# MatejBevec/gcn-song-embeddings

Hardware: AMD Instinct MI355X
Metric: PinSAGE train-step nodes/sec (2-hop, batch 512) at 1/2/4/8 MI355X (higher is better)
Workload: dtype f32

## Files before the change

### gcn-song-embeddings_amd/csrc/conv.hip

```cpp
#include "common.h"
#include "conv.h"
#include "bf16split.h"

#include <algorithm>
#include <climits>

namespace ps {

__device__ __forceinline__ int32_t rank_in(const unsigned long long* bits, const uint32_t* prefix,
                                           int64_t v) {
  const unsigned long long w = bits[v >> 6];
  return (int32_t)(prefix[v >> 6] + __popcll(w & ((1ull << (v & 63)) - 1ull)));
}

__global__ void layer_prep_kernel(LayerPreps a) {
  const int T = a.T;
  const int64_t g0 = (int64_t)blockIdx.x * blockDim.x + threadIdx.x, gs = (int64_t)gridDim.x * blockDim.x;
  for (int l = 0; l < a.n; ++l) {
    const LayerPrep& p = a.L[l];
    if (p.z) {
      const int64_t zn4 = (int64_t)(*p.z_rows) * p.z_n / 4;
      float4* z4 = reinterpret_cast<float4*>(p.z);
      for (int64_t i = g0; i < zn4; i += gs) z4[i] = make_float4(0.f, 0.f, 0.f, 0.f);
    }
// ... 383 lines not shown
  extern __shared__ int hist[];
  const int64_t n = (int64_t)(*nS) * T;
  const int U = *nN;
  const int ns = *nsplit;
  for (int si = blockIdx.x; si < ns; si += gridDim.x) {
    const int2 sp = split[si];
    const int v = off[sp.x + 1] - off[sp.x], nc = n_chunks(v);
    for (int j = threadIdx.x; j < nc; j += blockDim.x)
      chunks[sp.y + j] = make_int2(sp.x, min(kDqChunk, v - j * kDqChunk) | kDqSplit);
  }
  if (U <= kLdsRows) {
    for (int u = threadIdx.x; u < U; u += blockDim.x) hist[u] = 0;
    __syncthreads();
    const int64_t per = (n + gridDim.x - 1) / gridDim.x;
    const int64_t e0 = (int64_t)blockIdx.x * per, e1 = min(n, e0 + per);
    for (int64_t e = e0 + threadIdx.x; e < e1; e += blockDim.x) atomicAdd(hist + loc[e], 1);
    __syncthreads();
    for (int u = threadIdx.x; u < U; u += blockDim.x)
      if (hist[u]) hist[u] = atomicAdd(cursor + u, hist[u]);
    __syncthreads();
    for (int64_t e = e0 + threadIdx.x; e < e1; e += blockDim.x) {
      const int32_t u = loc[e];
      const int pos = atomicAdd(hist + u, 1);
      put_occ(occ2, off, cbase, wloc, T, u, pos, e);
    }
    return;
  }
  const int R = (U + kLdsRows - 1) / kLdsRows;
  if (R <= max_ranges) {
    const int64_t S = max((int64_t)1, (int64_t)(2 * gridDim.x + R - 1) / R);
    const int64_t slice = (n + S - 1) / S;
    const int64_t items = (int64_t)R * S;
    for (int64_t it = blockIdx.x; it < items; it += gridDim.x) {
      const int r = (int)(it % R);
      const int u0 = r * kLdsRows, nu = min(kLdsRows, U - u0);
      const int64_t e0 = (it / R) * slice, e1 = min(n, e0 + slice);
      for (int u = threadIdx.x; u < nu; u += blockDim.x) hist[u] = 0;
      __syncthreads();
      for (int64_t e = e0 + threadIdx.x; e < e1; e += blockDim.x) {
        const int u = loc[e] - u0;
        if ((unsigned)u < (unsigned)nu) atomicAdd(hist + u, 1);
      }
      __syncthreads();
      for (int u = threadIdx.x; u < nu; u += blockDim.x)
        if (hist[u]) hist[u] = atomicAdd(cursor + u0 + u, hist[u]);
      __syncthreads();
      for (int64_t e = e0 + threadIdx.x; e < e1; e += blockDim.x) {
        const int u = loc[e] - u0;
        if ((unsigned)u < (unsigned)nu) {
          const int pos = atomicAdd(hist + u, 1);
          put_occ(occ2, off, cbase, wloc, T, u0 + u, pos, e);
        }
      }
      __syncthreads();
    }
    return;
  }
  const int lane = threadIdx.x & 63;
  for (int64_t base = ((int64_t)blockIdx.x * blockDim.x + threadIdx.x) & ~63LL; base < n;
       base += (int64_t)gridDim.x * blockDim.x) {
    const int64_t e = base + lane;
    const int32_t u = e < n ? loc[e] : -1;
    unsigned long long rem = __ballot(e < n);
    int pos = 0;
    while (rem) {
      const int leader = __ffsll((long long)rem) - 1;
      const int32_t v = __shfl(u, leader, 64);
      const unsigned long long m = __ballot(u == v);
      int b = 0;
      if (lane == leader) b = atomicAdd(cursor + v, __popcll(m));
      b = __shfl(b, leader, 64);
      if (u == v) pos = b + __popcll(m & ((1ull << lane) - 1));
      rem &= ~m;
    }
    if (e < n) put_occ(occ2, off, cbase, wloc, T, u, pos, e);
  }
}

constexpr int kSortWaveRow = 64;
__global__ __launch_bounds__(256) void csr_sort_chunks_kernel(const int2* __restrict__ chunks,
                                                              const int* __restrict__ nchunks,
                                                              const int* __restrict__ off,
                                                              int2* __restrict__ occ2) {
  const int lane = threadIdx.x & 63;
  const int64_t nw = ((int64_t)gridDim.x * blockDim.x) >> 6;
  const int nch = *nchunks;
  for (int64_t ci = ((int64_t)blockIdx.x * blockDim.x + threadIdx.x) >> 6; ci < nch; ci += nw) {
    const int2 dsc = chunks[ci];
    const int n = dsc.y & 0xff;
    if (dsc.y & kDqSplit) {
      if (ci > 0 && chunks[ci - 1].x == dsc.x) continue;
      const int nr = off[dsc.x + 1] - off[dsc.x];
      if (nr > kSortWaveRow) continue;
      const int2 v = lane < nr ? occ2[ci * kDqChunk + lane] : make_int2(INT_MAX, 0);
      int r = 0;
      for (int j = 0; j < nr; ++j) r += __shfl(v.x, j, 64) < v.x;
      __builtin_amdgcn_wave_barrier();
      if (lane < nr) occ2[ci * kDqChunk + r] = v;
      continue;
    }
    if (n < 2) continue;
    int2 v = make_int2(INT_MAX, 0);
    if (lane < n) v = occ2[ci * kDqChunk + lane];
#pragma unroll
    for (int k = 2; k <= kDqChunk; k <<= 1)
#pragma unroll
      for (int j = k >> 1; j > 0; j >>= 1) {
        const int ox = __shfl_xor(v.x, j, 64), oy = __shfl_xor(v.y, j, 64);
        const bool lower = (lane & j) == 0, up = (lane & k) == 0;
        const bool take = (lower == up) ? (ox < v.x) : (ox > v.x);
        if (take) v = make_int2(ox, oy);
      }
    if (lane < n) occ2[ci * kDqChunk + lane] = v;
  }
}

constexpr int kRankWords = 16384;
constexpr int64_t kRankBits = (int64_t)kRankWords * 32;
constexpr int kRankLds = kRankWords * 4 * 2 + 64;
__global__ __launch_bounds__(1024) void csr_sort_rows_kernel(const int2* __restrict__ split,
                                                             const int* __restrict__ nsplit,
                                                             const int* __restrict__ off, int2* __restrict__ occ2,
                                                             int2* __restrict__ tmp) {
  extern __shared__ unsigned rk[];
  unsigned* bits = rk;
  unsigned* pref = rk + kRankWords;
  int* red = reinterpret_cast<int*>(pref + kRankWords);
  const int tid = threadIdx.x, lane = tid & 63, wv = tid >> 6;
  const int ns = *nsplit;
  for (int si = blockIdx.x; si < ns; si += gridDim.x) {
    const int2 sp = split[si];
    const int n = off[sp.x + 1] - off[sp.x];
    if (n <= kSortWaveRow) continue;
    int2* row = occ2 + (int64_t)sp.y * kDqChunk;
    int2* out = tmp + (int64_t)sp.y * kDqChunk;
    int lo = INT_MAX, hi = -1;
    for (int i = tid; i < n; i += blockDim.x) {
      const int f = row[i].x;
      lo = min(lo, f);
      hi = max(hi, f);
    }
    for (int o = 32; o > 0; o >>= 1) {
      lo = min(lo, __shfl_xor(lo, o, 64));
      hi = max(hi, __shfl_xor(hi, o, 64));
    }
    if (lane == 0) red[wv] = lo;
    __syncthreads();
    if (tid == 0) {
      int a = red[0];
      for (int w = 1; w < 16; ++w) a = min(a, red[w]);
      red[0] = a;
    }
    __syncthreads();
    lo = red[0];
    __syncthreads();
    if (lane == 0) red[wv] = hi;
    __syncthreads();
    if (tid == 0) {
      int a = red[0];
      for (int w = 1; w < 16; ++w) a = max(a, red[w]);
      red[0] = a;
    }
    __syncthreads();
    hi = red[0];
    __syncthreads();
    int base = 0;
    for (int64_t w0 = lo; w0 <= hi; w0 += kRankBits) {
      const int nwords = (int)min((int64_t)kRankWords, (hi - w0) / 32 + 1);
      for (int i = tid; i < nwords; i += blockDim.x) bits[i] = 0u;
      __syncthreads();
      for (int i = tid; i < n; i += blockDim.x) {
        const int64_t b = (int64_t)row[i].x - w0;
        if (b >= 0 && b < (int64_t)nwords * 32) atomicOr(bits + (b >> 5), 1u << (b & 31));
      }
      __syncthreads();
      const int per = (nwords + (int)blockDim.x - 1) / (int)blockDim.x;
      const int i0 = tid * per;
      int s = 0;
      for (int i = i0; i < min(nwords, i0 + per); ++i) s += __popc(bits[i]);
      int inc = s;
      for (int o = 1; o < 64; o <<= 1) {
        const int y = __shfl_up(inc, o, 64);
        if (lane >= o) inc += y;
      }
      if (lane == 63) red[wv] = inc;
      __syncthreads();
      int pre = inc - s;
      for (int w = 0; w < wv; ++w) pre += red[w];
      int total = 0;
      for (int w = 0; w < 16; ++w) total += red[w];
      for (int i = i0; i < min(nwords, i0 + per); ++i) {
        pref[i] = (unsigned)pre;
        pre += __popc(bits[i]);
      }
      __syncthreads();
      for (int i = tid; i < n; i += blockDim.x) {
        const int2 v = row[i];
        const int64_t b = (int64_t)v.x - w0;
        if (b >= 0 && b < (int64_t)nwords * 32) {
          const int wd = (int)(b >> 5);
          const int r = base + (int)pref[wd] + __popc(bits[wd] & ((1u << (b & 31)) - 1u));
          out[r] = v;
        }
      }
      base += total;
      __syncthreads();
    }
    __threadfence_block();
    __syncthreads();
    for (int i = tid; i < n; i += blockDim.x) row[i] = out[i];
    __syncthreads();
  }
}

typedef int dq_v4i __attribute__((ext_vector_type(4)));
__device__ __forceinline__ void dq_store_planes(uint16_t* __restrict__ base, int64_t ps, int64_t e, float4 v) {
  float a = v.x, b = v.y, c = v.z, d = v.w;
  asm("" : "+v"(a), "+v"(b), "+v"(c), "+v"(d));
  unsigned h0, m0, l0, h1, m1, l1;
  split_pair(f32x2{a, b}, h0, m0, l0);
  split_pair(f32x2{c, d}, h1, m1, l1);
  *reinterpret_cast<uint2*>(base + e) = make_uint2(h0, h1);
  *reinterpret_cast<uint2*>(base + ps + e) = make_uint2(m0, m1);
  *reinterpret_cast<uint2*>(base + 2 * ps + e) = make_uint2(l0, l1);
}
__device__ __forceinline__ void dq_st_wt(float* row, int i, float4 v) {
  const __amdgpu_buffer_rsrc_t rs = __builtin_amdgcn_make_buffer_rsrc(row, 0, 0x7fffffff, 0x00020000);
  const dq_v4i w{__float_as_int(v.x), __float_as_int(v.y), __float_as_int(v.z), __float_as_int(v.w)};
  __builtin_amdgcn_raw_buffer_store_b128(w, rs, (unsigned)i * 16u, 0, 16);
}
__device__ __forceinline__ float4 dq_ld_wt(const float* row, int i) {
  const __amdgpu_buffer_rsrc_t rs =
      __builtin_amdgcn_make_buffer_rsrc(const_cast<float*>(row), 0, 0x7fffffff, 0x00020000);
  const dq_v4i y = __builtin_amdgcn_raw_buffer_load_b128(rs, (unsigned)i * 16u, 0, 16);
  return make_float4(__int_as_float(y.x), __int_as_float(y.y), __int_as_float(y.z), __int_as_float(y.w));
}
template <int VEC, bool PL3>
__device__ __forceinline__ void dq_tree_leaf(float4 (&acc)[VEC], const float4 (&qv)[VEC], int u, int64_t ci,
                                             int lane, int h4, int hid, const int* __restrict__ off,
                                             const int* __restrict__ cbase, int* __restrict__ tk,
                                             int64_t tk_stride, float* __restrict__ part,
                                             float* __restrict__ dpq, uint16_t* __restrict__ dpq3,
                                             int64_t ps3) {
  const int k = n_chunks(off[u + 1] - off[u]);
  const int64_t cb = cbase[u];
  int64_t g = ci - cb, span = 1, nodes = k;
  float* leaf = part + (int64_t)__builtin_amdgcn_readfirstlane((int)ci) * hid;
#pragma unroll
  for (int v = 0; v < VEC; ++v)
    if (v * 64 + lane < h4) dq_st_wt(leaf, v * 64 + lane, acc[v]);
  for (int L = 0;; ++L) {
    asm volatile("s_waitcnt vmcnt(0)" ::: "memory");
    const int64_t gp = g >> 3;
    const int nch = (int)min<int64_t>(8, nodes - 8 * gp);
    int t = 0;
    if (lane == 0) t = __hip_atomic_fetch_add(tk + L * tk_stride + cb + gp, 1, __ATOMIC_RELAXED,
                                              __HIP_MEMORY_SCOPE_AGENT);
    t = __shfl(t, 0, 64);
    if (t != nch - 1) return;
    if (lane == 0) __hip_atomic_store(tk + L * tk_stride + cb + gp, 0, __ATOMIC_RELAXED, __HIP_MEMORY_SCOPE_AGENT);
    __builtin_amdgcn_fence(__ATOMIC_ACQUIRE, "wavefront");
    float4 x[8][VEC];
#pragma unroll
    for (int c = 0; c < 8; ++c) {
      const int cc = c < nch ? c : nch - 1;
      const float* row = part + (cb + span * (8 * gp + cc)) * hid;
#pragma unroll
      for (int v = 0; v < VEC; ++v) x[c][v] = dq_ld_wt(row, min(v * 64 + lane, h4 - 1));
    }
#pragma unroll
    for (int v = 0; v < VEC; ++v) acc[v] = x[0][v];
#pragma unroll
    for (int c = 1; c < 8; ++c)
      if (c < nch)
#pragma unroll
        for (int v = 0; v < VEC; ++v) {
          acc[v].x += x[c][v].x;
          acc[v].y += x[c][v].y;
          acc[v].z += x[c][v].z;
          acc[v].w += x[c][v].w;
        }
    span *= 8;
    nodes = (nodes + 7) >> 3;
    g = gp;
    if (nodes == 1) {
      float4* o = reinterpret_cast<float4*>(dpq + (int64_t)u * hid);
#pragma unroll
      for (int v = 0; v < VEC; ++v)
        if (v * 64 + lane < h4) {
          const float4 r = make_float4(acc[v].x * lrelu_grad(qv[v].x), acc[v].y * lrelu_grad(qv[v].y),
                                       acc[v].z * lrelu_grad(qv[v].z), acc[v].w * lrelu_grad(qv[v].w));
          if (PL3) dq_store_planes(dpq3, ps3, (int64_t)u * hid + 4 * (v * 64 + lane), r);
          else o[v * 64 + lane] = r;
        }
      return;
    }
    float* node = part + (int64_t)__builtin_amdgcn_readfirstlane((int)(cb + span * g)) * hid;
#pragma unroll
    for (int v = 0; v < VEC; ++v)
      if (v * 64 + lane < h4) dq_st_wt(node, v * 64 + lane, acc[v]);
  }
}

template <int VEC, bool CM = false, bool TREE = false, bool PL3 = false>
__global__ __launch_bounds__(256) void dq_chunk_kernel(
    const int2* __restrict__ chunks, const int* __restrict__ nchunks, const int2* __restrict__ occ2,
    const float* __restrict__ dagg, int64_t ld_dagg, const float* __restrict__ q, int hid,
    float* __restrict__ dpq, float* __restrict__ part, const int32_t* __restrict__ q_src = nullptr,
    int32_t* __restrict__ csrc = nullptr, const int* __restrict__ off = nullptr,
    const int* __restrict__ cbase = nullptr, int* __restrict__ tk = nullptr, int64_t tk_stride = 0,
    uint16_t* __restrict__ dpq3 = nullptr, int64_t ps3 = 0) {
  const int lane = threadIdx.x & 63;
  const int64_t wid = ((int64_t)blockIdx.x * blockDim.x + threadIdx.x) >> 6;
  const int64_t nw = ((int64_t)gridDim.x * blockDim.x) >> 6;
  const int h4 = hid >> 2;
  const int nch = *nchunks;
  int2 dsc = make_int2(0, 0), oc = make_int2(0, 0);
  if (wid < nch) {
    dsc = chunks[wid];
    if (lane < kDqChunk) oc = occ2[wid * kDqChunk + lane];
  }
  if (!CM && h4 <= 64 * VEC) {
    float4 pend[VEC];
    float4* pend_o = nullptr;
    int64_t pend_e = -1;
    auto store_pend = [&]() __attribute__((always_inline)) {
      if (PL3 && pend_e >= 0) {
#pragma unroll
        for (int v = 0; v < VEC; ++v)
          if (v * 64 + lane < h4) dq_store_planes(dpq3, ps3, pend_e + 4 * (v * 64 + lane), pend[v]);
        pend_e = -1;
      } else if (pend_o) {
#pragma unroll
        for (int v = 0; v < VEC; ++v)
          if (v * 64 + lane < h4) pend_o[v * 64 + lane] = pend[v];
        pend_o = nullptr;
      }
    };
    for (int64_t ci = wid; ci < nch; ci += nw) {
      int2 dsc_n = make_int2(0, 0), oc_n = make_int2(0, 0);
      if (ci + nw < nch) {
        dsc_n = chunks[ci + nw];
        if (lane < kDqChunk) oc_n = occ2[(ci + nw) * kDqChunk + lane];
      }
      const int u = dsc.x, n = dsc.y & 0xff;
      const bool split = (dsc.y & kDqSplit) != 0;
      const int32_t my_row = oc.x;
      const float my_w = __int_as_float(oc.y);
      float4 qv[VEC], x[kDqChunk][VEC];
#pragma unroll
      for (int v = 0; v < VEC; ++v) qv[v] = reinterpret_cast<const float4*>(q + (int64_t)u * hid)[min(v * 64 + lane, h4 - 1)];
      const int ng = (n + 3) >> 2;
#pragma unroll
      for (int g = 0; g < kDqChunk / 4; ++g) {
        if (g < ng) {
#pragma unroll
          for (int jj = 0; jj < 4; ++jj) {
            const int j = 4 * g + jj;
            const int32_t row = __shfl(my_row, min(j, n - 1), 64);
            const float4* dr = reinterpret_cast<const float4*>(dagg + (int64_t)row * ld_dagg);
#pragma unroll
            for (int v = 0; v < VEC; ++v) x[j][v] = dr[min(v * 64 + lane, h4 - 1)];
          }
        }
      }
      store_pend();
      float4 acc[VEC];
#pragma unroll
      for (int v = 0; v < VEC; ++v) acc[v] = make_float4(0.f, 0.f, 0.f, 0.f);
#pragma unroll
      for (int g = 0; g < kDqChunk / 4; ++g) {
        if (g < ng) {
#pragma unroll
          for (int jj = 0; jj < 4; ++jj) {
            const int j = 4 * g + jj;
            const float w = j < n ? __shfl(my_w, j, 64) : 0.f;
#pragma unroll
            for (int v = 0; v < VEC; ++v) {
              acc[v].x = fmaf(w, x[j][v].x, acc[v].x);
              acc[v].y = fmaf(w, x[j][v].y, acc[v].y);
              acc[v].z = fmaf(w, x[j][v].z, acc[v].z);
              acc[v].w = fmaf(w, x[j][v].w, acc[v].w);
            }
          }
        }
      }
      if (TREE && split) {
        dq_tree_leaf<VEC, PL3>(acc, qv, u, ci, lane, h4, hid, off, cbase, tk, tk_stride, part, dpq, dpq3, ps3);
        dsc = dsc_n;
        oc = oc_n;
        continue;
      }
#pragma unroll
      for (int v = 0; v < VEC; ++v)
        pend[v] = split ? acc[v]
                        : make_float4(acc[v].x * lrelu_grad(qv[v].x), acc[v].y * lrelu_grad(qv[v].y),
                                      acc[v].z * lrelu_grad(qv[v].z), acc[v].w * lrelu_grad(qv[v].w));
      if (PL3 && !split) pend_e = (int64_t)u * hid;
      else pend_o = reinterpret_cast<float4*>(split ? part + ci * hid : dpq + (int64_t)u * hid);
      dsc = dsc_n;
      oc = oc_n;
    }
    store_pend();
    return;
  }
  for (int64_t ci = wid; ci < nch; ci += nw) {
    int2 dsc_n = make_int2(0, 0), oc_n = make_int2(0, 0);
    if (ci + nw < nch) {
      dsc_n = chunks[ci + nw];
      if (lane < kDqChunk) oc_n = occ2[(ci + nw) * kDqChunk + lane];
    }
    const int u = dsc.x, n = dsc.y & 0xff;
    const bool split = !CM && (dsc.y & kDqSplit) != 0;
    if (CM && lane == 0) csrc[ci] = q_src[u];
    const int32_t my_row = oc.x;
    const float my_w = __int_as_float(oc.y);
    for (int c0 = 0; c0 < h4; c0 += 64 * VEC) {
      float4 qv[VEC], x[kDqChunk][VEC];
#pragma unroll
      for (int v = 0; v < VEC; ++v) {
        const int c = min(c0 + v * 64 + lane, h4 - 1);
        qv[v] = reinterpret_cast<const float4*>(q + (int64_t)u * hid)[c];
      }
      const int ng = (n + 3) >> 2;
#pragma unroll
      for (int g = 0; g < kDqChunk / 4; ++g) {
        if (g < ng) {
#pragma unroll
          for (int jj = 0; jj < 4; ++jj) {
            const int j = 4 * g + jj;
            const int32_t row = __shfl(my_row, min(j, n - 1), 64);
            const float4* dr = reinterpret_cast<const float4*>(dagg + (int64_t)row * ld_dagg);
#pragma unroll
            for (int v = 0; v < VEC; ++v) x[j][v] = dr[min(c0 + v * 64 + lane, h4 - 1)];
          }
        }
      }
      float4 acc[VEC];
#pragma unroll
      for (int v = 0; v < VEC; ++v) acc[v] = make_float4(0.f, 0.f, 0.f, 0.f);
#pragma unroll
      for (int g = 0; g < kDqChunk / 4; ++g) {
        if (g < ng) {
#pragma unroll
          for (int jj = 0; jj < 4; ++jj) {
            const int j = 4 * g + jj;
            const float w = j < n ? __shfl(my_w, j, 64) : 0.f;
#pragma unroll
            for (int v = 0; v < VEC; ++v) {
              acc[v].x = fmaf(w, x[j][v].x, acc[v].x);
              acc[v].y = fmaf(w, x[j][v].y, acc[v].y);
              acc[v].z = fmaf(w, x[j][v].z, acc[v].z);
              acc[v].w = fmaf(w, x[j][v].w, acc[v].w);
            }
          }
        }
      }
      float4* o = reinterpret_cast<float4*>(split || CM ? part + ci * hid : dpq + (int64_t)u * hid);
#pragma unroll
      for (int v = 0; v < VEC; ++v) {
        const int c = c0 + v * 64 + lane;
        if (c < h4)
          o[c] = split ? acc[v]
                       : make_float4(acc[v].x * lrelu_grad(qv[v].x), acc[v].y * lrelu_grad(qv[v].y),
                                     acc[v].z * lrelu_grad(qv[v].z), acc[v].w * lrelu_grad(qv[v].w));
      }
    }
    dsc = dsc_n;
    oc = oc_n;
  }
}

constexpr int kCombWaves = 16;
__global__ __launch_bounds__(1024) void dq_combine_kernel(const int2* __restrict__ split,
                                                          const int* __restrict__ nsplit,
                                                          const int* __restrict__ off,
                                                          const float* __restrict__ part,
                                                          const float* __restrict__ q, int hid,
                                                          float* __restrict__ dpq) {
  __shared__ float4 red[kCombWaves][64];
  const int lane = threadIdx.x & 63, wv = threadIdx.x >> 6;
  const int h4 = hid >> 2;
  const int ns = *nsplit;
  for (int si = blockIdx.x; si < ns; si += gridDim.x) {
    const int2 sp = split[si];
    const int u = sp.x;
    const int64_t ci = sp.y;
    const int k = (off[u + 1] - off[u] + kDqChunk - 1) / kDqChunk;
    for (int c0 = 0; c0 < h4; c0 += 64) {
      const int c = c0 + lane;
      const int cc = min(c, h4 - 1);
      float4 acc = make_float4(0.f, 0.f, 0.f, 0.f);
      int j = wv;
      for (; j + 7 * kCombWaves < k; j += 8 * kCombWaves) {
        float4 x[8];
#pragma unroll
        for (int i = 0; i < 8; ++i)
          x[i] = reinterpret_cast<const float4*>(part + (ci + j + i * kCombWaves) * hid)[cc];
#pragma unroll
        for (int i = 0; i < 8; ++i) {
          acc.x += x[i].x;
          acc.y += x[i].y;
          acc.z += x[i].z;
          acc.w += x[i].w;
        }
      }
      for (; j < k; j += kCombWaves) {
        const float4 x = reinterpret_cast<const float4*>(part + (ci + j) * hid)[cc];
        acc.x += x.x;
        acc.y += x.y;
        acc.z += x.z;
        acc.w += x.w;
      }
      red[wv][lane] = acc;
      __syncthreads();
      if (wv == 0 && c < h4) {
        float4 t = red[0][lane];
        for (int i = 1; i < kCombWaves; ++i) {
          const float4 x = red[i][lane];
          t.x += x.x;
          t.y += x.y;
          t.z += x.z;
          t.w += x.w;
        }
        const float4 qq = reinterpret_cast<const float4*>(q + (int64_t)u * hid)[c];
        reinterpret_cast<float4*>(dpq + (int64_t)u * hid)[c] =
            make_float4(t.x * lrelu_grad(qq.x), t.y * lrelu_grad(qq.y), t.z * lrelu_grad(qq.z),
                        t.w * lrelu_grad(qq.w));
      }
      __syncthreads();
    }
  }
}

__global__ __launch_bounds__(256) void norm_lrelu_bwd_kernel(const float* __restrict__ y,
                                                             const float* __restrict__ nrm,
                                                             const float* __restrict__ dy, int n,
                                                             const int* __restrict__ nrows,
                                                             int64_t n_static,
                                                             float* __restrict__ dp,
                                                             float* __restrict__ z, int z_n,
                                                             const int* __restrict__ z_rows,
                                                             int* __restrict__ zi, int64_t zi_n) {
  const int64_t gt = (int64_t)blockIdx.x * blockDim.x + threadIdx.x;
  const int64_t gs = (int64_t)gridDim.x * blockDim.x;
  const int64_t R = nrows ? (int64_t)*nrows : n_static;
  const int lane = threadIdx.x & 63;
  const int64_t wid = ((int64_t)blockIdx.x * blockDim.x + threadIdx.x) >> 6;
  const int64_t nw = ((int64_t)gridDim.x * blockDim.x) >> 6;
  for (int64_t r = wid; r < R; r += nw) {
    float dot = 0.f;
    for (int c = lane; c < n; c += 64) dot += y[r * n + c] * dy[r * n + c];
    dot = wave_sum(dot);
    const float inv = 1.f / nrm[r];
    for (int c = lane; c < n; c += 64) {
      const float yy = y[r * n + c];
      dp[r * n + c] = lrelu_grad(yy) * (dy[r * n + c] - yy * dot) * inv;
    }
  }
  if (z) {
    const int64_t zn = (int64_t)(*z_rows) * z_n;
    for (int64_t i = gt; i < zn; i += gs) z[i] = 0.f;
  }
  if (zi)
    for (int64_t i = gt; i < zi_n; i += gs) zi[i] = 0;
}

__global__ __launch_bounds__(256) void l2norm_rows_kernel(float* __restrict__ y, int64_t n, int out,
                                                          float* __restrict__ norms) {
  const int lane = threadIdx.x & 63;
  const int64_t wid = ((int64_t)blockIdx.x * blockDim.x + threadIdx.x) >> 6;
  const int64_t nw = ((int64_t)gridDim.x * blockDim.x) >> 6;
  for (int64_t r = wid; r < n; r += nw) {
    float s2 = 0.f;
    for (int c = lane; c < out; c += 64) s2 += y[r * out + c] * y[r * out + c];
    const float nrm = sqrtf(wave_sum(s2));
    for (int c = lane; c < out; c += 64) y[r * out + c] = y[r * out + c] / nrm;
    if (lane == 0 && norms) norms[r] = nrm;
  }
}

int launch_l2norm_rows(float* y, int64_t n, int out, float* norms, hipStream_t st) {
  if (n <= 0) return kOk;
  hipLaunchKernelGGL(l2norm_rows_kernel, dim3(grid_for(n * 64, 256, 4096)), dim3(256), 0, st, y, n, out, norms);
  PS_CHECK_LAUNCH();
  return kOk;
}

constexpr int kPosCsrMax = 16384;
constexpr int kPosDig = 7, kPosBuckets = 1 << kPosDig, kPosWaves = 16;
constexpr int kPosCsrLds = 2 * kPosCsrMax * 4 + kPosBuckets * kPosWaves * 4 + 64;
__device__ __forceinline__ unsigned long long match_digit(int dig, bool valid) {
  unsigned long long m = __ballot(valid);
#pragma unroll
  for (int bit = 0; bit < kPosDig; ++bit) {
    const unsigned long long bb = __ballot((dig >> bit) & 1);
    m &= ((dig >> bit) & 1) ? bb : ~bb;
  }
  return m;
}
__global__ __launch_bounds__(1024) void pos_csr_kernel(const int32_t* __restrict__ pos_rank, int n,
                                                       const int* __restrict__ nS, int* __restrict__ rank_off,
                                                       int32_t* __restrict__ pos_sorted) {
  extern __shared__ unsigned pk[];
  if (n > kPosCsrMax) {
    if (threadIdx.x == 0) rank_off[0] = -1;
    return;
  }
  unsigned* src = pk;
  unsigned* dst = pk + kPosCsrMax;
  int* base = reinterpret_cast<int*>(pk + 2 * kPosCsrMax);
  int* wsum = base + kPosBuckets * kPosWaves;
  const int tid = threadIdx.x, lane = tid & 63, wv = tid >> 6;
  for (int i = tid; i < n; i += blockDim.x) src[i] = ((unsigned)pos_rank[i] << 16) | (unsigned)i;
  const int seg = ((n + kPosWaves - 1) / kPosWaves + 63) & ~63;
  const int w0 = min(n, wv * seg), w1 = min(n, w0 + seg);
  const unsigned long long below = (1ull << lane) - 1ull;
  for (int pass = 0; pass < 2; ++pass) {
    const int sh = 16 + kPosDig * pass;
    for (int i = tid; i < kPosBuckets * kPosWaves; i += blockDim.x) base[i] = 0;
    __syncthreads();
    for (int i0 = w0; i0 < w1; i0 += 64) {
      const int i = i0 + lane;
      const bool valid = i < w1;
      const int dig = valid ? (int)(src[i] >> sh) & (kPosBuckets - 1) : 0;
      const unsigned long long m = match_digit(dig, valid);
      if (valid && (m & below) == 0) base[dig * kPosWaves + wv] += __popcll(m);
    }
    __syncthreads();
    const int c0 = base[2 * tid], c1 = base[2 * tid + 1];
    int inc = c0 + c1;
    for (int o = 1; o < 64; o <<= 1) {
      const int y = __shfl_up(inc, o, 64);
      if (lane >= o) inc += y;
    }
    if (lane == 63) wsum[wv] = inc;
    __syncthreads();
    int pre = inc - c0 - c1;
    for (int w = 0; w < wv; ++w) pre += wsum[w];
    base[2 * tid] = pre;
    base[2 * tid + 1] = pre + c0;
    __syncthreads();
    for (int i0 = w0; i0 < w1; i0 += 64) {
      const int i = i0 + lane;
      const bool valid = i < w1;
      const unsigned key = valid ? src[i] : 0u;
      const int dig = (int)(key >> sh) & (kPosBuckets - 1);
      const unsigned long long m = match_digit(dig, valid);
      const int b = valid ? base[dig * kPosWaves + wv] : 0;
      __builtin_amdgcn_wave_barrier();
      if (valid) {
        dst[b + __popcll(m & below)] = key;
        if ((m & below) == 0) base[dig * kPosWaves + wv] = b + __popcll(m);
      }
      __builtin_amdgcn_wave_barrier();
    }
    __syncthreads();
    unsigned* t = src;
    src = dst;
    dst = t;
  }
  for (int i = tid; i < n; i += blockDim.x) {
    const unsigned v = src[i];
    const int r = (int)(v >> 16);
    pos_sorted[i] = (int32_t)(v & 0xffffu);
    const int rp = i == 0 ? -1 : (int)(src[i - 1] >> 16);
    for (int q = rp + 1; q <= r; ++q) rank_off[q] = i;
  }
  const int qe = max(*nS, (int)(src[n - 1] >> 16) + 1);
  for (int q = (int)(src[n - 1] >> 16) + 1 + tid; q <= qe; q += blockDim.x) rank_off[q] = n;
}

int launch_pos_csr(const int32_t* pos_rank, int64_t n, const int* nS, int* rank_off, int32_t* pos_sorted,
                   hipStream_t st) {
  static bool prepared = false;
  if (!prepared) {
    PS_CHECK_HIP(hipFuncSetAttribute((const void*)pos_csr_kernel, hipFuncAttributeMaxDynamicSharedMemorySize,
                                     kPosCsrLds));
    prepared = true;
  }
  if (n <= 0) return kOk;
  hipLaunchKernelGGL(pos_csr_kernel, dim3(1), dim3(1024), n <= kPosCsrMax ? (unsigned)kPosCsrLds : 0u, st, pos_rank,
                     (int)std::min<int64_t>(n, INT32_MAX), nS, rank_off, pos_sorted);
  PS_CHECK_LAUNCH();
  return kOk;
}

__device__ __forceinline__ int det_mode(int ro0, int a0, int a1) { return ro0 < 0 ? -1 : a1 - a0 == 1 ? 0 : 1; }
template <int XPL>
__device__ __forceinline__ void det_put(const float (&x)[XPL], int d, int p, int r, int grp, int mode,
                                        float* __restrict__ G, int64_t S_max, float* __restrict__ Gp, int lane) {
  float* g = G + ((int64_t)grp * S_max + r) * d;
  if (mode < 0) {
#pragma unroll
    for (int i = 0; i < XPL; ++i)
      if (lane + 64 * i < d) atomicAdd(g + lane + 64 * i, x[i]);
    return;
  }
  float* dst = mode == 0 ? g : Gp + (int64_t)p * d;
#pragma unroll
  for (int i = 0; i < XPL; ++i)
    if (lane + 64 * i < d) dst[lane + 64 * i] = x[i];
}

constexpr int kRepBatch = 16;
template <int XPL, int NG>
__global__ __launch_bounds__(256) void rep_sum_kernel(const int* __restrict__ rank_off,
                                                      const int32_t* __restrict__ pos_sorted,
                                                      const int* __restrict__ nS, int d,
                                                      const float* __restrict__ Gp, float* __restrict__ G,
                                                      int64_t S_max) {
  if (rank_off[0] < 0) return;
  const int lane = threadIdx.x & 63;
  const int64_t nw = ((int64_t)gridDim.x * blockDim.x) >> 6;
  const int64_t R = *nS;
  for (int64_t r = ((int64_t)blockIdx.x * blockDim.x + threadIdx.x) >> 6; r < R; r += nw) {
    const int o0 = rank_off[r], o1 = rank_off[r + 1];
    if (o1 - o0 < 2) continue;
    float acc[NG][XPL];
    bool any[NG];
#pragma unroll
    for (int c = 0; c < NG; ++c) {
      any[c] = false;
#pragma unroll
      for (int i = 0; i < XPL; ++i) acc[c][i] = 0.f;
    }
    for (int o = o0; o < o1; o += kRepBatch) {
      const int my_q = lane < kRepBatch && o + lane < o1 ? pos_sorted[o + lane] : -1;
      int q[kRepBatch];
      float v[kRepBatch][XPL];
#pragma unroll
      for (int u = 0; u < kRepBatch; ++u) q[u] = __shfl(my_q, u, 64);
#pragma unroll
      for (int u = 0; u < kRepBatch; ++u)
#pragma unroll
        for (int i = 0; i < XPL; ++i)
          v[u][i] = q[u] >= 0 && lane + 64 * i < d ? Gp[(int64_t)q[u] * d + lane + 64 * i] : 0.f;
#pragma unroll
      for (int u = 0; u < kRepBatch; ++u) {
        if (q[u] < 0) continue;
        const int c = NG == 1 ? 0 : q[u] % NG;
#pragma unroll
        for (int cc = 0; cc < NG; ++cc)
          if (cc == c) {
            any[cc] = true;
#pragma unroll
            for (int i = 0; i < XPL; ++i) acc[cc][i] += v[u][i];
          }
      }
    }
#pragma unroll
    for (int c = 0; c < NG; ++c)
      if (any[c]) {
        float* g = G + ((int64_t)c * S_max + r) * d;
#pragma unroll
        for (int i = 0; i < XPL; ++i)
          if (lane + 64 * i < d) g[lane + 64 * i] = acc[c][i];
      }
  }
}
// ... 794 lines not shown
```

Measured before the change: 4.154 million.

## Double-buffer dq chunk row loads and specialize on group count

Rewrites the dq chunk accumulation as a helper that keeps only two groups of four gathered rows in registers. It issues the next group's loads while FMAs run on the current group, and dispatches on the group count so each variant is fully unrolled without runtime branches. Row indices and weights move to scalar readlane/readfirstlane instead of shfl, and launch bounds now request higher occupancy. The aim is to cut VGPR pressure and hide gather latency; the risk is register spills under the tighter bound or a worse schedule from the sched barriers.

```diff
diff --git a/gcn-song-embeddings_amd/csrc/conv.hip b/gcn-song-embeddings_amd/csrc/conv.hip
--- a/gcn-song-embeddings_amd/csrc/conv.hip
+++ b/gcn-song-embeddings_amd/csrc/conv.hip
@@ -709,8 +709,69 @@
   }
 }
 
+template <int VEC, int NG, class F>
+__device__ __forceinline__ void dq_chunk_sum(float4 (&acc)[VEC], const float* __restrict__ dagg, int64_t ld_dagg,
+                                             int2 oc, int n, int c0, int lane, int h4, F&& behind_loads) {
+  float4 x[2][4][VEC];
+  unsigned col[VEC];
+  const int wbits = lane < n ? oc.y : 0;
+#pragma unroll
+  for (int v = 0; v < VEC; ++v) col[v] = 16u * (unsigned)min(c0 + v * 64 + lane, h4 - 1);
+  auto issue = [&](int g) __attribute__((always_inline)) {
+#pragma unroll
+    for (int jj = 0; jj < 4; ++jj) {
+      const int32_t row = __builtin_amdgcn_readlane(oc.x, min(4 * g + jj, n - 1));
+      const char* dr = reinterpret_cast<const char*>(dagg + (int64_t)row * ld_dagg);
+#pragma unroll
+      for (int v = 0; v < VEC; ++v) x[g & 1][jj][v] = *reinterpret_cast<const float4*>(dr + col[v]);
+    }
+  };
+  issue(0);
+  if (NG > 1) issue(1);
+  behind_loads();
+#pragma unroll
+  for (int v = 0; v < VEC; ++v) acc[v] = make_float4(0.f, 0.f, 0.f, 0.f);
+#pragma unroll
+  for (int g = 0; g < NG; ++g) {
+#pragma unroll
+    for (int jj = 0; jj < 4; ++jj) {
+      const float w = __int_as_float(__builtin_amdgcn_readlane(wbits, 4 * g + jj));
+#pragma unroll
+      for (int v = 0; v < VEC; ++v) {
+        acc[v].x = fmaf(w, x[g & 1][jj][v].x, acc[v].x);
+        acc[v].y = fmaf(w, x[g & 1][jj][v].y, acc[v].y);
+        acc[v].z = fmaf(w, x[g & 1][jj][v].z, acc[v].z);
+        acc[v].w = fmaf(w, x[g & 1][jj][v].w, acc[v].w);
+      }
+    }
+    if (g + 2 < NG) {
+#pragma unroll
+      for (int v = 0; v < VEC; ++v)
+        asm volatile("" : "+v"(acc[v].x), "+v"(acc[v].y), "+v"(acc[v].z), "+v"(acc[v].w), "+v"(col[v]));
+      issue(g + 2);
+      __builtin_amdgcn_sched_barrier(0);
+    }
+  }
+}
+template <int VEC, class F>
+__device__ __forceinline__ void dq_chunk_sum_n(float4 (&acc)[VEC], const float* __restrict__ dagg, int64_t ld_dagg,
+                                               int2 oc, int n, int c0, int lane, int h4, F&& behind_loads) {
+  static_assert(kDqChunk <= 16 && kDqChunk % 4 == 0, "dq: chunks are 1 to 4 groups of 4 rows");
+  switch ((n + 3) >> 2) {
+    case 0:
+#pragma unroll
+      for (int v = 0; v < VEC; ++v) acc[v] = make_float4(0.f, 0.f, 0.f, 0.f);
+      behind_loads();
+      break;
+    case 1: dq_chunk_sum<VEC, 1>(acc, dagg, ld_dagg, oc, n, c0, lane, h4, behind_loads); break;
+    case 2: dq_chunk_sum<VEC, 2>(acc, dagg, ld_dagg, oc, n, c0, lane, h4, behind_loads); break;
+    case 3: dq_chunk_sum<VEC, 3>(acc, dagg, ld_dagg, oc, n, c0, lane, h4, behind_loads); break;
+    default: dq_chunk_sum<VEC, 4>(acc, dagg, ld_dagg, oc, n, c0, lane, h4, behind_loads); break;
+  }
+}
+
 template <int VEC, bool CM = false, bool TREE = false, bool PL3 = false>
-__global__ __launch_bounds__(256) void dq_chunk_kernel(
+__global__ __launch_bounds__(256, (PL3 && VEC > 1) ? 3 : 4) void dq_chunk_kernel(
     const int2* __restrict__ chunks, const int* __restrict__ nchunks, const int2* __restrict__ occ2,
     const float* __restrict__ dagg, int64_t ld_dagg, const float* __restrict__ q, int hid,
     float* __restrict__ dpq, float* __restrict__ part, const int32_t* __restrict__ q_src = nullptr,
@@ -718,7 +779,8 @@
     const int* __restrict__ cbase = nullptr, int* __restrict__ tk = nullptr, int64_t tk_stride = 0,
     uint16_t* __restrict__ dpq3 = nullptr, int64_t ps3 = 0) {
   const int lane = threadIdx.x & 63;
-  const int64_t wid = ((int64_t)blockIdx.x * blockDim.x + threadIdx.x) >> 6;
+  const int64_t wid =
+      __builtin_amdgcn_readfirstlane((int)(((int64_t)blockIdx.x * blockDim.x + threadIdx.x) >> 6));
   const int64_t nw = ((int64_t)gridDim.x * blockDim.x) >> 6;
   const int h4 = hid >> 2;
   const int nch = *nchunks;
@@ -750,48 +812,13 @@
         dsc_n = chunks[ci + nw];
         if (lane < kDqChunk) oc_n = occ2[(ci + nw) * kDqChunk + lane];
       }
-      const int u = dsc.x, n = dsc.y & 0xff;
-      const bool split = (dsc.y & kDqSplit) != 0;
-      const int32_t my_row = oc.x;
-      const float my_w = __int_as_float(oc.y);
-      float4 qv[VEC], x[kDqChunk][VEC];
+      const int u = __builtin_amdgcn_readfirstlane(dsc.x), dy = __builtin_amdgcn_readfirstlane(dsc.y);
+      const int n = dy & 0xff;
+      const bool split = (dy & kDqSplit) != 0;
+      float4 qv[VEC], acc[VEC];
 #pragma unroll
       for (int v = 0; v < VEC; ++v) qv[v] = reinterpret_cast<const float4*>(q + (int64_t)u * hid)[min(v * 64 + lane, h4 - 1)];
-      const int ng = (n + 3) >> 2;
-#pragma unroll
-      for (int g = 0; g < kDqChunk / 4; ++g) {
-        if (g < ng) {
-#pragma unroll
-          for (int jj = 0; jj < 4; ++jj) {
-            const int j = 4 * g + jj;
-            const int32_t row = __shfl(my_row, min(j, n - 1), 64);
-            const float4* dr = reinterpret_cast<const float4*>(dagg + (int64_t)row * ld_dagg);
-#pragma unroll
-            for (int v = 0; v < VEC; ++v) x[j][v] = dr[min(v * 64 + lane, h4 - 1)];
-          }
-        }
-      }
-      store_pend();
-      float4 acc[VEC];
-#pragma unroll
-      for (int v = 0; v < VEC; ++v) acc[v] = make_float4(0.f, 0.f, 0.f, 0.f);
-#pragma unroll
-      for (int g = 0; g < kDqChunk / 4; ++g) {
-        if (g < ng) {
-#pragma unroll
-          for (int jj = 0; jj < 4; ++jj) {
-            const int j = 4 * g + jj;
-            const float w = j < n ? __shfl(my_w, j, 64) : 0.f;
-#pragma unroll
-            for (int v = 0; v < VEC; ++v) {
-              acc[v].x = fmaf(w, x[j][v].x, acc[v].x);
-              acc[v].y = fmaf(w, x[j][v].y, acc[v].y);
-              acc[v].z = fmaf(w, x[j][v].z, acc[v].z);
-              acc[v].w = fmaf(w, x[j][v].w, acc[v].w);
-            }
-          }
-        }
-      }
+      dq_chunk_sum_n<VEC>(acc, dagg, ld_dagg, oc, n, 0, lane, h4, store_pend);
       if (TREE && split) {
         dq_tree_leaf<VEC, PL3>(acc, qv, u, ci, lane, h4, hid, off, cbase, tk, tk_stride, part, dpq, dpq3, ps3);
         dsc = dsc_n;
@@ -817,52 +844,18 @@
       dsc_n = chunks[ci + nw];
       if (lane < kDqChunk) oc_n = occ2[(ci + nw) * kDqChunk + lane];
     }
-    const int u = dsc.x, n = dsc.y & 0xff;
-    const bool split = !CM && (dsc.y & kDqSplit) != 0;
+    const int u = __builtin_amdgcn_readfirstlane(dsc.x), dy = __builtin_amdgcn_readfirstlane(dsc.y);
+    const int n = dy & 0xff;
+    const bool split = !CM && (dy & kDqSplit) != 0;
     if (CM && lane == 0) csrc[ci] = q_src[u];
-    const int32_t my_row = oc.x;
-    const float my_w = __int_as_float(oc.y);
     for (int c0 = 0; c0 < h4; c0 += 64 * VEC) {
-      float4 qv[VEC], x[kDqChunk][VEC];
+      float4 qv[VEC], acc[VEC];
 #pragma unroll
       for (int v = 0; v < VEC; ++v) {
         const int c = min(c0 + v * 64 + lane, h4 - 1);
         qv[v] = reinterpret_cast<const float4*>(q + (int64_t)u * hid)[c];
       }
-      const int ng = (n + 3) >> 2;
-#pragma unroll
-      for (int g = 0; g < kDqChunk / 4; ++g) {
-        if (g < ng) {
-#pragma unroll
-          for (int jj = 0; jj < 4; ++jj) {
-            const int j = 4 * g + jj;
-            const int32_t row = __shfl(my_row, min(j, n - 1), 64);
-            const float4* dr = reinterpret_cast<const float4*>(dagg + (int64_t)row * ld_dagg);
-#pragma unroll
-            for (int v = 0; v < VEC; ++v) x[j][v] = dr[min(c0 + v * 64 + lane, h4 - 1)];
-          }
-        }
-      }
-      float4 acc[VEC];
-#pragma unroll
-      for (int v = 0; v < VEC; ++v) acc[v] = make_float4(0.f, 0.f, 0.f, 0.f);
-#pragma unroll
-      for (int g = 0; g < kDqChunk / 4; ++g) {
-        if (g < ng) {
-#pragma unroll
-          for (int jj = 0; jj < 4; ++jj) {
-            const int j = 4 * g + jj;
-            const float w = j < n ? __shfl(my_w, j, 64) : 0.f;
-#pragma unroll
-            for (int v = 0; v < VEC; ++v) {
-              acc[v].x = fmaf(w, x[j][v].x, acc[v].x);
-              acc[v].y = fmaf(w, x[j][v].y, acc[v].y);
-              acc[v].z = fmaf(w, x[j][v].z, acc[v].z);
-              acc[v].w = fmaf(w, x[j][v].w, acc[v].w);
-            }
-          }
-        }
-      }
+      dq_chunk_sum_n<VEC>(acc, dagg, ld_dagg, oc, n, c0, lane, h4, [] {});
       float4* o = reinterpret_cast<float4*>(split || CM ? part + ci * hid : dpq + (int64_t)u * hid);
 #pragma unroll
       for (int v = 0; v < VEC; ++v) {
```

Measured after the change: 4.191 million (median of 6 runs). No clear change (+0.9%).
